# 14chanwa/remotesensingProject

Hardware: AMD Instinct MI355X
Metric: Mpixel*disparity-hypotheses/s (higher is better)
Workload: dtype f32

## Files before the change

### remotesensingproject_amd/csrc/k2_reg.hpp

```cpp
#pragma once

#include "k2_scan.hpp"
#include "k2_taps.hpp"

namespace rslf {

#ifndef RSLF_REG_GB104
#define RSLF_REG_GB104 8
#endif
constexpr int gather_batch(int c) { return c == 1 ? 8 : 4; }
constexpr int kPadSlack = 16;

template <int SPAD, int C, bool PK, bool KONLY>
__device__ __forceinline__ void mean_shift_pass(const float (&R)[PK ? 1 : C][PK ? 1 : SPAD], const f2 (&R2)[PK ? C : 1][PK ? SPAD / 2 : 1],
                                                int S, float kq, const float (&rbar)[C], float (&A)[C], float& B)
{
    static_assert(!KONLY || (C == 1 && !PK), "the K-only pass is written for the scalar one-channel blocks");
    if constexpr (PK) {
        f2 rb2[C];
        const f2 kq2 = {kq, kq};
#pragma unroll
        for (int c = 0; c < C; c++)
            rb2[c] = f2{rbar[c], rbar[c]};
        constexpr int kBlk = (C == 1) ? 8 : 4;
#pragma unroll
        for (int s0 = 0; s0 < SPAD; s0 += kBlk) {
            if (!(s0 < SPAD - kPadSlack || s0 < S))
                continue;
            if constexpr (C == 1) {
                f2 P[4], K[4];
                const f2 r4[4] = {R2[0][s0 / 2], R2[0][s0 / 2 + 1], R2[0][s0 / 2 + 2], R2[0][s0 / 2 + 3]};
                mean_shift_pk_octet(r4, rb2[0], kq2, P, K);
#pragma unroll
                for (int j = 0; j < 4; j++) {
                    A[0] = A[0] + P[j].x;
                    B = B + K[j].x;
                    A[0] = A[0] + P[j].y;
                    B = B + K[j].y;
                }
            } else {
                f2 Pa[3], Pb[3], Ka, Kb;
                const f2 ra[3] = {R2[0][s0 / 2], R2[1][s0 / 2], R2[C - 1][s0 / 2]};
                const f2 rb[3] = {R2[0][s0 / 2 + 1], R2[1][s0 / 2 + 1], R2[C - 1][s0 / 2 + 1]};
                const f2 m[3] = {rb2[0], rb2[C > 1 ? 1 : 0], rb2[C - 1]};
                mean_shift_pk_rgb_quad(ra, rb, m, kq2, Pa, Pb, Ka, Kb);
#pragma unroll
                for (int c = 0; c < C; c++)
                    A[c] = A[c] + Pa[c].x;
                B = B + Ka.x;
#pragma unroll
                for (int c = 0; c < C; c++)
                    A[c] = A[c] + Pa[c].y;
                B = B + Ka.y;
#pragma unroll
                for (int c = 0; c < C; c++)
                    A[c] = A[c] + Pb[c].x;
                B = B + Kb.x;
#pragma unroll
                for (int c = 0; c < C; c++)
                    A[c] = A[c] + Pb[c].y;
                B = B + Kb.y;
            }
        }
    } else if (C == 1) {
#pragma unroll
        for (int s0 = 0; s0 < SPAD; s0 += 4) {
            if (s0 + 4 <= SPAD - kPadSlack || s0 + 4 <= S) {
                if constexpr (KONLY)
                    mean_shift_group4_k(R[0][s0], R[0][s0 + 1], R[0][s0 + 2], R[0][s0 + 3], rbar[0], kq, B);
                else
                    mean_shift_group4(R[0][s0], R[0][s0 + 1], R[0][s0 + 2], R[0][s0 + 3], rbar[0], kq, A[0], B);
            } else {
#pragma unroll
                for (int j = 0; j < 3; j++)
                    if (s0 + j < S) {
                        if constexpr (KONLY)
                            mean_shift_group1_k(R[0][s0 + j], rbar[0], kq, B);
                        else
                            mean_shift_group1(R[0][s0 + j], rbar[0], kq, A[0], B);
                    }
            }
        }
    } else {
#pragma unroll
        for (int s = 0; s < SPAD; s++) {
            if (!(s < SPAD - kPadSlack || s < S))
                continue;
            float q[C];
#pragma unroll
            for (int c = 0; c < C; c++) {
                const float delta = R[c][s] - rbar[c];
                const float tq = kq * delta;
                q[c] = tq * delta;
            }
            float qs = q[0];
            if (C == 3) {
                qs = q[0] + q[C - 1];
                qs = qs + q[C > 1 ? 1 : 0];
            }
            const float K = kernel_weight(qs);
#pragma unroll
            for (int c = 0; c < C; c++) {
                const float pr = R[c][s] * K;
                A[c] = A[c] + pr;
            }
            B = B + K;
        }
    }
}

template <int SPAD, int C, int BATCH>
__device__ __forceinline__ void tap_table_batch(const float* epi, const float* otab, const int* tboff, const f2* tw, unsigned du_bytes,
                                                float uf, int S, int stride_s, bool from_table, int g, int& rowoff, float (&R)[C][SPAD])
{
    float tt[BATCH], om[BATCH], e0[C][BATCH], e1[C][BATCH];
    unsigned bo[BATCH];
    if (from_table) {
#pragma unroll
        for (int j = 0; j < BATCH; j++) {
            const int s = g * BATCH + j;
            bo[j] = (unsigned)tboff[s] + du_bytes;
            const f2 w = tw[s];
            tt[j] = w.x;
            om[j] = w.y;
        }
    } else {
        int ro = rowoff;
#pragma unroll
        for (int j = 0; j < BATCH; j++) {
            const int s = g * BATCH + j;
            tt[j] = 0.0f;
            bo[j] = 0;
            if (s < SPAD - kPadSlack || s < S) {
                const float x = otab[s] + uf;
                tt[j] = lerp_weight(x);
                const int i0 = floor_to_int(x);
                bo[j] = (unsigned)(i0 * C + ro) << 2;
            }
            om[j] = 1.0f - tt[j];
            ro += stride_s;
        }
    }
    rowoff += BATCH * stride_s;
#pragma unroll
    for (int j = 0; j < BATCH; j++) {
        const int s = g * BATCH + j;
#pragma unroll
        for (int c = 0; c < C; c++) {
            e0[c][j] = kSentinel;
            e1[c][j] = 0.0f;
        }
        if (s < SPAD - kPadSlack || s < S) {
            const float* p = (const float*)((const char*)epi + bo[j]);
#pragma unroll
            for (int c = 0; c < C; c++) {
                e0[c][j] = p[c];
                e1[c][j] = p[C + c];
            }
        }
    }
#pragma unroll
    for (int j = 0; j < BATCH; j++) {
        const int s = g * BATCH + j;
#pragma unroll
        for (int c = 0; c < C; c++) {
            const float m0 = om[j] * e0[c][j];
            const float m1 = tt[j] * e1[c][j];
            const float r = m0 + m1;
            R[c][s] = (s < SPAD - kPadSlack || s < S) ? r : kSentinel;
        }
    }
}

template <int SPAD, int C, bool BORDER, bool UNIFORM_D, bool PK, int GB = 0, class BestT = Best<C>, bool LANE_D = false,
          bool TRIM = false, bool TAPS = false>
__device__ __forceinline__ void scan_reg_body(const ScanArgs& a, int v, int u, int d0, int d1, BestT& best,
                                              float* __restrict__ otab, int dlane = 0, int dstep = 1)
{
    static_assert(!LANE_D || !UNIFORM_D, "hypotheses in the lanes: every lane has its own view offsets");
    constexpr int kGatherBatch = GB > 0 ? GB : (C == 1 && !PK && SPAD == 104 && RSLF_REG_GB104 == 13) ? 13 : gather_batch(C);
    static_assert(SPAD % kGatherBatch == 0 && (!PK || kGatherBatch % 2 == 0), "whole batches, whole pairs");
    static_assert(SPAD % 8 == 0, "slot counts are multiples of 8");
    static_assert(!TAPS || (UNIFORM_D && !BORDER && !PK), "the tap table belongs to the interior scalar uniform-D row form");
    const VolView& vol = a.vol;
    const float* epi = vol.row(v, 0);
    const float uf = (float)u;
    const int Um1 = vol.U - 1;
    const unsigned Um1_bits = __float_as_uint((float)Um1);
    const int S = vol.S;
    const int lane = threadIdx.x & 63;
    const long long o = (long long)v * vol.U + u;
    const float dmin = a.dmin_vu ? a.dmin_vu[o] : a.dmin;
    const float dmax = a.dmax_vu ? a.dmax_vu[o] : a.dmax;
    const float range = dmax - dmin;
    const float denom = (float)(a.dim_d - 1);
    const float kq = (C == 1) ? a.k.k1 : a.k.inv_h2;
    const float slope = a.k.slope;
    const int stride_s = (int)vol.stride_s;
    float centre[C];
#pragma unroll
    for (int c = 0; c < C; c++)
        centre[c] = epi[(long long)a.s_hat * vol.stride_s + u * C + c];
    int* const tboff = TAPS ? reinterpret_cast<int*>(otab + SPAD) : nullptr;
    f2* const tw = TAPS ? reinterpret_cast<f2*>(otab + 2 * SPAD) : nullptr;
    int u_first = 0, u_last = 0;
    unsigned du_bytes = 0;
    bool taps_on = false;
    if constexpr (TAPS) {
        u_first = __builtin_amdgcn_readfirstlane(u);
        u_last = __builtin_amdgcn_readlane(u, 63);
        const int du = u - u_first;
        du_bytes = (unsigned)(du * C) << 2;
        taps_on = a.tap_table != 0 && __all(du == min(lane, u_last - u_first));
    }

#pragma unroll 1
    for (int dk = d0; dk < d1; dk += (LANE_D ? dstep : 1)) {
        const int d = LANE_D ? min(dk + dlane, d1 - 1) : dk;
        const float Dd = hypothesis(dmin, range, denom, d);
        float R[PK ? 1 : C][PK ? 1 : SPAD];
        f2 R2[PK ? C : 1][PK ? SPAD / 2 : 1];
        int card = BORDER ? 0 : S;
        float Ss0 = (float)a.s_hat;
        asm volatile("" : "+v"(Ss0));
        int rowoff = 0;
        asm volatile("" : "+s"(rowoff));
        unsigned fastb = 0;
        if (UNIFORM_D) {
            int lane_s = lane, tile_first = u_first, tile_last = u_last;
            if constexpr (TAPS)
                asm volatile("" : "+v"(lane_s), "+s"(tile_first), "+s"(tile_last));
#pragma unroll
            for (int s0 = 0; s0 < SPAD; s0 += 64) {
                const int s = s0 + lane_s;
                float off = (float)(a.s_hat - s) * Dd;
                off = off * slope;
                if (SPAD % 64 == 0 || s < SPAD)
                    otab[s] = off;
                if constexpr (TAPS) {
                    if (taps_on) {
                        const TapEntry e = tap_entry(off, tile_first, tile_last, vol.U, C, __mul24(s, stride_s));
                        if (SPAD % 64 == 0 || s < SPAD) {
                            tboff[s] = e.byteoff;
                            tw[s] = f2{e.t, e.omt};
                        }
                        unsigned long long m = __ballot(e.fast);
                        m &= m >> 1;
                        m &= m >> 2;
                        m &= m >> 4;
                        static_assert(!TAPS || kGatherBatch == 8, "the batch bits are gathered for batches of eight samples");
#pragma unroll
                        for (int k = 0; k < 8; k++)
                            if (s0 + 8 * k < SPAD)
                                fastb |= ((unsigned)(m >> (8 * k)) & 1u) << (s0 / 8 + k);
                    }
                }
            }
            __builtin_amdgcn_wave_barrier();
            if constexpr (TAPS)
                fastb = __builtin_amdgcn_readfirstlane(fastb & (S >= SPAD ? ~0u : (1u << (S / kGatherBatch)) - 1u));
        }
#pragma unroll
        for (int g = 0; g < SPAD / kGatherBatch; g++) {
            if constexpr (TAPS) {
                tap_table_batch<SPAD, C, kGatherBatch>(epi, otab, tboff, tw, du_bytes, uf, S, stride_s, (fastb >> g) & 1u, g, rowoff, R);
            } else {
                float tt[kGatherBatch], e0[C][kGatherBatch], e1[C][kGatherBatch];
                bool ok[kGatherBatch];
#pragma unroll
                for (int j = 0; j < kGatherBatch; j++) {
                    const int s = g * kGatherBatch + j;
                    tt[j] = 0.0f;
                    ok[j] = false;
#pragma unroll
                    for (int c = 0; c < C; c++) {
                        e0[c][j] = kSentinel;
                        e1[c][j] = 0.0f;
                    }
                    if (s < SPAD - kPadSlack || s < S) {
                        float x;
                        if (UNIFORM_D) {
                            x = otab[s];
                        } else {
                            x = (Ss0 - (float)s) * Dd;
                            x = x * slope;
                        }
                        x = x + uf;
                        tt[j] = lerp_weight(x);
                        int i0 = floor_to_int(x);
                        ok[j] = true;
                        if (BORDER) {
                            ok[j] = __float_as_uint(x) <= Um1_bits;
                            i0 = ok[j] ? i0 : 0;
                        }
                        const unsigned byteoff = (unsigned)(i0 * C + rowoff) << 2;
                        const float* p = (const float*)((const char*)epi + byteoff);
#pragma unroll
                        for (int c = 0; c < C; c++) {
                            e0[c][j] = p[c];
                            e1[c][j] = p[C + c];
                        }
                    }
                    rowoff += stride_s;
                }
#pragma unroll
                for (int j = 0; j < kGatherBatch; j++) {
                    const int s = g * kGatherBatch + j;
                    const float omt = 1.0f - tt[j];
#pragma unroll
                    for (int c = 0; c < C; c++) {
                        const float m0 = omt * e0[c][j];
                        const float m1 = tt[j] * e1[c][j];
                        const float r = m0 + m1;
                        float val;
                        if (BORDER)
                            val = ok[j] ? r : kSentinel;
                        else
                            val = (s < SPAD - kPadSlack || s < S) ? r : kSentinel;
                        if constexpr (PK) {
                            if (s & 1)
                                R2[c][s >> 1].y = val;
                            else
                                R2[c][s >> 1].x = val;
                        } else {
                            R[c][s] = val;
                        }
                    }
                    if (BORDER)
                        card += ok[j] ? 1 : 0;
                }
            }
            {
                const int b = g * kGatherBatch;
#pragma unroll
                for (int c = 0; c < C; c++) {
                    if constexpr (PK) {
                        asm volatile("" : "+v"(R2[c][b / 2]), "+v"(R2[c][b / 2 + 1]));
                        if (kGatherBatch == 8)
                            asm volatile("" : "+v"(R2[c][b / 2 + 2]), "+v"(R2[c][b / 2 + 3]));
                        static_assert(!PK || kGatherBatch == 4 || kGatherBatch == 8, "pair pinning is written for 4 and 8");
                    } else if (kGatherBatch != 4 && kGatherBatch != 8) {
#pragma unroll
                        for (int j = 0; j < kGatherBatch; j++)
                            asm volatile("" : "+v"(R[c][b + j]));
                    } else {
                        asm volatile("" : "+v"(R[c][b + 0]), "+v"(R[c][b + 1]), "+v"(R[c][b + 2]), "+v"(R[c][b + 3]));
                        if (kGatherBatch == 8)
                            asm volatile("" : "+v"(R[c][b + kGatherBatch - 4]), "+v"(R[c][b + kGatherBatch - 3]),
                                              "+v"(R[c][b + kGatherBatch - 2]), "+v"(R[c][b + kGatherBatch - 1]));
                    }
                }
                if (BORDER)
                    asm volatile("" : "+s"(rowoff), "+v"(Ss0), "+v"(card));
                else
                    asm volatile("" : "+s"(rowoff), "+v"(Ss0));
            }
        }

        float rbar[C];
#pragma unroll
        for (int c = 0; c < C; c++)
            rbar[c] = centre[c];
        float B = 0.0f;
#pragma unroll 1
        for (int it = 0; it < a.k.n_iter; it++) {
            float A[C];
#pragma unroll
            for (int c = 0; c < C; c++)
                A[c] = 0.0f;
            B = 0.0f;
            if constexpr (TRIM) {
                if (it == a.k.n_iter - 1) {
                    mean_shift_pass<SPAD, C, PK, true>(R, R2, S, kq, rbar, A, B);
                    break;
                }
            }
            mean_shift_pass<SPAD, C, PK, false>(R, R2, S, kq, rbar, A, B);
#pragma unroll
            for (int c = 0; c < C; c++) {
                const float qd = (B != 0.0f) ? (A[c] / B) : 0.0f;
                rbar[c] = (qd > 0.0f) ? qd : 0.0f;
            }
        }
        const float cardf = (float)card;
        float sc = (card != 0) ? (B / cardf) : 0.0f;
        sc = (sc > 0.0f) ? sc : 0.0f;
        if (!LANE_D || dk + dlane < d1)
            best.offer(sc, d, Dd, rbar);
    }
}

template <int C>
struct LastPassRbar {
    __device__ __forceinline__ void operator()(const ScanArgs& a, long long o, float Dd, float (&rbar)[C]) const
    {
        if (a.k.n_iter == 0)
            return;
        const VolView& vol = a.vol;
        const int v = (int)(o / vol.U);
        const int u = (int)(o - (long long)v * vol.U);
        const float* epi = vol.row(v, 0);
        const float uf = (float)u;
        const unsigned Um1_bits = __float_as_uint((float)(vol.U - 1));
        const float kq = (C == 1) ? a.k.k1 : a.k.inv_h2;
        const float Ss0 = (float)a.s_hat;
        const int S = vol.S;
        float A[C];
#pragma unroll
        for (int c = 0; c < C; c++)
            A[c] = 0.0f;
// ... 88 lines not shown
#ifndef RSLF_TAP_TABLE
#define RSLF_TAP_TABLE 1
#endif
constexpr bool scan_reg_tap_table(int spad, int c) { return RSLF_TAP_TABLE && c == 1 && spad == 104 && scan_reg_trim(spad, c); }

template <int SPAD, int C>
using ScanRegRbarFix = std::conditional_t<scan_reg_trim(SPAD, C), LastPassRbar<C>, NoRbarFix>;

template <int SPAD, int C, class BestT>
__device__ __forceinline__ void scan_reg_rows(const ScanArgs& a, int v, int u, int d0, int d1, BestT& best, float* otab)
{
    constexpr bool PK = scan_reg_packed_math(SPAD, C);
    constexpr bool kTaps = scan_reg_tap_table(SPAD, C);
    if (a.dmin_vu) {
        scan_reg_body<SPAD, C, true, false, PK, 0, BestT, false, scan_reg_trim(SPAD, C)>(a, v, u, d0, d1, best, otab);
        return;
    }
    const float max_ds = (float)max(a.s_hat, a.vol.S - 1 - a.s_hat);
    const float range = a.dmax - a.dmin, denom = (float)(a.dim_d - 1);
    const float uf = (float)u, Um1 = (float)(a.vol.U - 1);
    auto interior = [&](int d) -> bool {
        const float reach = max_ds * fabsf(hypothesis(a.dmin, range, denom, d)) * fabsf(a.k.slope) + 2.0f;
        return __all((uf - reach >= 0.0f) && (uf + reach <= Um1));
    };
    int d = d0;
    while (d < d1) {
        const bool in = interior(d);
        int e = d + 1;
        while (e < d1 && interior(e) == in)
            e++;
        if (in)
            scan_reg_body<SPAD, C, false, true, PK, 0, BestT, false, scan_reg_trim(SPAD, C), kTaps>(a, v, u, d, e, best, otab);
        else
            scan_reg_body<SPAD, C, true, true, PK, 0, BestT, false, scan_reg_trim(SPAD, C)>(a, v, u, d, e, best, otab);
        d = e;
    }
}

template <int SPAD, int C>
__global__ __launch_bounds__(64 * kScanWaves) __attribute__((amdgpu_waves_per_eu(scan_reg_waves(SPAD, C), scan_reg_waves(SPAD, C))))
void k2_scan_reg(ScanArgs a)
{
    __shared__ __attribute__((aligned(16))) float s_otab[kScanWaves][SPAD * (scan_reg_tap_table(SPAD, C) ? 4 : 1)];
    float* otab = s_otab[__builtin_amdgcn_readfirstlane(threadIdx.x >> 6)];
    constexpr bool kEpiDyn = false;
    float* const epi_lds = nullptr;
    const int epi_stride = 0;
    using Fix = ScanRegRbarFix<SPAD, C>;
    if constexpr (scan_reg_best_in_lds(SPAD, C)) {
        __shared__ float s_best[kScanWaves][BestLds<C>::kFloats];
        BestLds<C> running(s_best[__builtin_amdgcn_readfirstlane(threadIdx.x >> 6)]);
        RSLF_SCAN_ROW_TILE_FIX((running.init(), scan_reg_rows<SPAD, C>(a, v, u, d0, d1, running, otab), running.load(best)), Fix{})
    } else {
        RSLF_SCAN_ROW_TILE_FIX((scan_reg_rows<SPAD, C>(a, v, u, d0, d1, best, otab)), Fix{})
    }
}

#ifndef RSLF_PACKED_LONG_GB
#define RSLF_PACKED_LONG_GB 4
#endif
constexpr bool packed_long_unit(int spad, int c) { return c == 1 && spad >= 80 && spad <= 128 && spad % RSLF_PACKED_LONG_GB == 0; }
constexpr int packed_waves(int spad, int c) { return packed_long_unit(spad, c) ? 2 : scan_reg_waves(spad + 24, c); }
constexpr int packed_gather_batch(int spad, int c) { return packed_long_unit(spad, c) ? spad / RSLF_PACKED_LONG_GB : 0; }

template <int SPAD, int C>
__global__ __launch_bounds__(64 * kScanWaves) __attribute__((amdgpu_waves_per_eu(packed_waves(SPAD, C), packed_waves(SPAD, C))))
void k2_scan_reg_packed(ScanArgs a)
// ... 48 lines not shown
```

### remotesensingproject_amd/csrc/k2_taps.hpp

```cpp
#pragma once

#include <math.h>
#include <stdint.h>
#include <string.h>

#if defined(__HIPCC__)
#define RSLF_TAPS_FN __host__ __device__ __forceinline__
#else
#define RSLF_TAPS_FN inline
#endif

namespace rslf {

struct TapEntry {
    int byteoff;
    float t, omt;
    bool fast;
};

RSLF_TAPS_FN uint32_t tap_float_bits(float x)
{
#if defined(__HIP_DEVICE_COMPILE__)
    return __float_as_uint(x);
#else
    uint32_t b;
    memcpy(&b, &x, sizeof(b));
    return b;
#endif
}

RSLF_TAPS_FN float tap_fract(float x)
{
#if defined(__HIP_DEVICE_COMPILE__)
    return __builtin_amdgcn_fractf(x);
#else
    return x - floorf(x);
#endif
}
RSLF_TAPS_FN int tap_floor(float x)
{
#if defined(__HIP_DEVICE_COMPILE__)
    int i;
    asm("v_cvt_flr_i32_f32_e32 %0, %1" : "=v"(i) : "v"(x));
    return i;
#else
    return (int)floorf(x);
#endif
}

RSLF_TAPS_FN TapEntry tap_entry(float off, int u_first, int u_last, int U, int C, int row_floats)
{
    const float uf = (float)u_first, ul = (float)u_last;
    const float x_first = off + uf;
    const float x_last = off + ul;
    TapEntry e;
    e.t = tap_fract(x_first);
    const int i0 = tap_floor(x_first);
    e.omt = 1.0f - e.t;
    e.byteoff = (int)((unsigned)(i0 * C + row_floats) << 2);
    const bool inside = x_first > 0.0f && x_last <= (float)(U - 1);
    const bool binade = ((tap_float_bits(x_first) ^ tap_float_bits(x_last)) >> 23) == 0;
    const float back = x_last - ul;
    const bool exact = back == off;
    e.fast = inside && (binade || exact);
    return e;
}

}
```

### remotesensingproject_amd/csrc/rslf_core.hip

```cpp
#include "rslf_internal.hpp"

#include <algorithm>
#include <cmath>

#include "k0_pack.hpp"

using namespace rslf;


namespace rslf {

char* last_error_buffer()
{
    static thread_local char g_err[512] = "";
    return g_err;
}

static std::atomic<int> g_inject[kInjectSites];

bool inject_hit(InjectSite site)
{
    std::atomic<int>& c = g_inject[site];
    int v = c.load(std::memory_order_relaxed);
    while (v > 0)
// ... 184 lines not shown
        (void)hipEventDestroy(ctx->ev1);
    delete ctx;
    return RSLF_OK;
}
RSLF_API_CATCH

extern "C" int rslf_ctx_set_stream(rslf_ctx* ctx, void* hip_stream) RSLF_API_TRY
{
    if (!ctx)
        return fail(RSLF_ERR_INVALID_ARG, "ctx is NULL");
    ctx->stream = (hipStream_t)hip_stream;
    return RSLF_OK;
}
RSLF_API_CATCH

extern "C" int rslf_ctx_set_debug(rslf_ctx* ctx, const char* key, int value) RSLF_API_TRY
{
    if (!ctx || !key)
        return fail(RSLF_ERR_INVALID_ARG, "ctx/key is NULL");
    if (strcmp(key, "force_scan") == 0 && value >= 0 && value <= 2)
        ctx->force_scan = value;
    else if (strcmp(key, "force_groups") == 0 && value >= 0 && value <= 64)
        ctx->force_groups = value;
    else if (strcmp(key, "force_packed") == 0 && value >= -1 && value <= 1)
        ctx->force_packed = value;
    else if (strcmp(key, "px") == 0 && value >= -1 && value <= 1)
        ctx->px_mode = value;
    else if (strcmp(key, "stream_share") == 0 && value >= 0 && value <= 2)
        ctx->stream_share = value;
    else if (strcmp(key, "row_split") == 0 && value >= 0 && value <= 65536)
        ctx->row_split = value;
    else if (strcmp(key, "tap_table") == 0 && (value == 0 || value == 1))
        ctx->tap_table = value;
    else if (strcmp(key, "claim_skip") == 0 && (value == 0 || value == 1))
        ctx->claim_skip = value;
    else if (strcmp(key, "time_all") == 0 && (value == 0 || value == 1)) {
        ctx->time_all = value;
        ctx->ev_used = 0;
    } else if (strcmp(key, "stream_groups") == 0 && value >= 0 && value <= 64)
        ctx->stream_groups = value;
    else if (strcmp(key, "stream_lds_kib") == 0 && value >= 16 && value <= 152) {
        ctx->stream_lds_bytes = (size_t)value << 10;
    } else if (strcmp(key, "staging_kib") == 0 && value >= 0 && value <= 262144)
        ctx->staging_kib = value;
    else
        return fail(RSLF_ERR_INVALID_ARG, "rslf_ctx_set_debug: unknown key or value out of range: %s = %d", key, value);
    return RSLF_OK;
}
RSLF_API_CATCH

extern "C" int rslf_ctx_synchronize(rslf_ctx* ctx) RSLF_API_TRY
{
    if (!ctx)
        return fail(RSLF_ERR_INVALID_ARG, "ctx is NULL");
    HIP_TRY(hipSetDevice(ctx->device));
    HIP_TRY(hipStreamSynchronize(ctx->stream));
    return RSLF_OK;
}
RSLF_API_CATCH


extern "C" int rslf_volume_create(rslf_ctx* ctx, int V, int S, int U, int C, rslf_volume** out) RSLF_API_TRY
{
    if (!ctx || !out)
        return fail(RSLF_ERR_INVALID_ARG, "ctx/out is NULL");
    *out = nullptr;
// ... 474 lines not shown
```

### remotesensingproject_amd/csrc/rslf_internal.hpp

```cpp
#pragma once

#include "../../include/rslf_hip.h"

#include <hip/hip_runtime.h>

#include <atomic>
#include <cstdarg>
#include <cstdio>
#include <cstring>
#include <exception>
#include <functional>
#include <memory>
#include <new>
#include <string>
#include <thread>
#include <vector>

#include "rslf_device.hpp"
#include "rslf_plan.hpp"
#include "rslf_scratch.hpp"


namespace rslf {

// ... 161 lines not shown
    int32_t* lc_idx_vu = nullptr;
    const float* lc_Ce_svu = nullptr;
    const float* lc_dmin_vu = nullptr;
    const float* lc_dmax_vu = nullptr;
    float lc_dmin = 0.0f, lc_dmax = 0.0f;
    int lc_dim_d = 0;
    ScanConsts lc_consts = {};
};

}

struct rslf_ctx {
    int device = 0;
    hipStream_t stream = nullptr;
    rslf::Scratch scratch;
    rslf::SweepState sweep;
    hipEvent_t ev0 = nullptr, ev1 = nullptr;
    bool ev_valid = false;
    int time_all = 0;
    std::vector<hipEvent_t> ev_pool;
    size_t ev_used = 0;
    int last_spad = 0;
    int last_kernel = 0;
    int num_cus = 0;
    int force_scan = 0;
    int force_groups = 0;
    int force_packed = -1;
    int px_mode = -1;
    int stream_groups = 0;
    int stream_share = 1;
    size_t stream_lds_bytes = rslf::plan::kStreamLdsBytes;
    int row_split = 1;
    int tap_table = 1;
    int claim_skip = 1;
    int staging_kib = 0;
};

struct rslf_volume {
    rslf_ctx* ctx = nullptr;
    int device = 0;
    int V = 0, S = 0, U = 0, C = 0, pitch = 0;
    float* base = nullptr;
    size_t bytes = 0;
    float min_value = 0.0f, max_value = 0.0f;
    bool filled = false;
};

struct rslf_multi {
    struct Dev {
        rslf_ctx* ctx = nullptr;
        hipStream_t s_up = nullptr, s_comp = nullptr, s_down = nullptr;
        hipEvent_t done[2] = {nullptr, nullptr};
        rslf_volume* vol[2] = {nullptr, nullptr};
        rslf::DeviceBuf planes[2];
        rslf::PinnedBuf pin[2];
        rslf::DeviceBuf arena;
    };
    std::vector<Dev> devs;
    int chunk_rows = 0;
    std::vector<unsigned char> peer;
};

namespace rslf {

struct StreamScope {
    StreamScope(rslf_ctx* ctx_, hipStream_t stream) : ctx(ctx_), saved(ctx_->stream) { ctx->stream = stream; }
// ... 133 lines not shown
```

### remotesensingproject_amd/csrc/rslf_pile.hip

```cpp
#include "rslf_internal.hpp"

#include <algorithm>
#include <cmath>

#include "k1_edge.hpp"
#include "k2_scan.hpp"
#include "k2_reg.hpp"
#include "k2_stream.hpp"
#include "k3_median.hpp"

using namespace rslf;

static_assert(sizeof(Partial) == plan::kPartialRecordBytes, "rslf_plan.hpp sizes the record scratch");
static_assert(kScanWaves == plan::kScanWavesPerTile, "rslf_plan.hpp shares the hypotheses out over this many waves");


extern "C" int rslf_edge_confidence_pile(rslf_ctx* ctx, const rslf_volume* vol, int s, const rslf_params* p,
                                         float* d_Ce_vu, uint8_t* d_Ce_mask_vu) RSLF_API_TRY
{
    if (!ctx || !vol || !d_Ce_vu || !d_Ce_mask_vu)
        return fail(RSLF_ERR_INVALID_ARG, "NULL argument");
    int rc = check_params(p);
    if (rc)
        return rc;
// ... 122 lines not shown
#define RSLF_C 3
            RSLF_SPAD_LIST_3CH(RSLF_CASE)
#undef RSLF_C
        default:
            break;
        }
    }
#undef RSLF_CASE
    return fail(RSLF_ERR_UNSUPPORTED, "no register scan kernel with %d slots x %d channels", spad, C);
}

static plan::ScanKernelFacts kernel_facts(int S, int C)
{
    const int spad = plan::pick_spad(S, C);
    return plan::ScanKernelFacts{spad ? scan_reg_waves(spad, C) : 0, stream_resident_for(S, C), stream_px_resident_for(S, C)};
}

static plan::ScanRequest scan_request(const rslf_ctx* ctx, int V, int U, int S, int C, int dim_d, bool in_range, bool linear,
                                      bool pixel_ranges, const ScanInputs& in)
{
    plan::ScanRequest rq = {};
    rq.V = V, rq.U = U, rq.S = S, rq.C = C, rq.dim_d = dim_d;
    rq.num_cus = ctx->num_cus;
    rq.ctx_groups = in.groups;
    rq.ctx_packed = in.packed;
    rq.precompacted = in.lists;
    rq.force_groups = ctx->force_groups;
    rq.force_packed = ctx->force_packed;
    rq.px_mode = ctx->px_mode;
    rq.stream_groups = ctx->stream_groups;
    rq.stream_share = ctx->stream_share;
    rq.stream_lds_bytes = ctx->stream_lds_bytes;
    rq.tap_table = ctx->tap_table;
    const bool dense_uniform = !pixel_ranges && !in.packed && ctx->force_packed != 1 && in.lists != ScanInputs::kPackedList;
    plan::choose_scan_kernel(&rq, in_range, linear, ctx->force_scan, dense_uniform, kernel_facts(S, C));
    return rq;
}

int rslf::scan_presize(rslf_ctx* ctx, int S, int U, int C, int dim_d, const rslf_params* p, const int* rows, int n_rows)
{
    const plan::ScanKernelFacts f = kernel_facts(S, C);
    int max_rows = 0;
    size_t recs = 0, tickets = 0;
    for (int i = 0; i < n_rows; i++) {
        max_rows = std::max(max_rows, rows[i]);
        ScanInputs in;
        if (p && plan::fuse_k1_compaction(p->edge_confidence_opening_size, ctx->force_packed, (size_t)rows[i] * U))
            in.lists = ScanInputs::kRowLists;
        const plan::ScanRequest rq = scan_request(ctx, rows[i], U, S, C, dim_d, true, !p || p->interpolation == RSLF_INTERP_LINEAR, false, in);
        const plan::ScanPlan sp = plan::plan_scan(rq, f.nres, f.nres_px);
        recs = std::max(recs, sp.records);
        tickets = std::max(tickets, sp.tickets);
    }
    if (max_rows < 1)
        return RSLF_OK;
    HIP_TRY(hipSetDevice(ctx->device));
    bool tickets_fresh = false;
    int rc = ensure_plane_scratch(ctx, max_rows, U);
    if (rc == RSLF_OK && recs)
        rc = ensure_group_scratch(ctx, recs, tickets, &tickets_fresh);
    if (rc == RSLF_OK && tickets_fresh)
        HIP_TRY(hipStreamSynchronize(ctx->stream));
    return rc;
}

int rslf::sweep_scan_presize(rslf_ctx* ctx, const rslf_volume* vol, int dim_d, const ScanInputs& sparse)
// ... 462 lines not shown
```

### remotesensingproject_amd/csrc/rslf_plan.hpp

```cpp
#pragma once

#include <stddef.h>
#include <stdint.h>

#include <string.h>

#include <algorithm>
#include <cmath>
#include <vector>

#include "../../include/rslf_hip.h"

namespace rslf {

struct MorphElement {
    int k;
    unsigned rows[31];
};

namespace plan {


constexpr int kScanWavesPerTile = 4;
constexpr size_t kPartialRecordBytes = 32;
// ... 547 lines not shown
inline int px_waves(int dim_d)
{
    int best = 0;
    double best_use = 0.0;
    for (int w = 1; w <= kScanWavesPerTile; w *= 2) {
        const int lanes = 64 * w, iters = (dim_d + lanes - 1) / lanes;
        const double use = (double)dim_d / ((double)iters * lanes);
        if (use >= best_use - 1e-12) {
            best_use = use;
            best = w;
        }
    }
    return best_use >= 0.6 ? best : 0;
}

struct ScanRequest {
    int V, U, S, C, dim_d;
    int spad;
    bool use_stream;
    bool use_chip;
    int chip_wave_floats;
    int reg_waves;
    int num_cus;
    int ctx_groups;
    bool ctx_packed;
    int precompacted;
    int force_groups;
    int force_packed;
    int px_mode;
    int stream_groups;
    int stream_share;
    size_t stream_lds_bytes;
    int tap_table;
};

struct ScanPlan {
    int kind;
    int spad;
    int groups;
    bool packed;
    bool packed_adapt;
    int px_waves;
    int tap_table;
    int tile_w;
    int tiles_per_row;
    int rows_per_launch;
    size_t records;
    size_t tickets;
    int stream_nres;
    int stream_park;
    int stream_wave_floats;
    size_t lds_bytes;
};

inline int stream_resident_hi(int C, int nres_1ch, int nres_rgb) { return C == 1 ? nres_1ch : nres_rgb; }

struct ScanKernelFacts {
    int reg_waves;
    int nres;
    int nres_px;
};

inline bool scan_range_ok(float min_value, float max_value) { return min_value >= 0.0f && max_value <= 1.0e6f; }

inline void choose_scan_kernel(ScanRequest* r, bool in_range, bool linear, int force_scan, bool dense_uniform, const ScanKernelFacts& f)
{
// ... 51 lines not shown
    if (r.force_packed >= 0)
        packed = r.force_packed != 0;
    if (n > (size_t)INT32_MAX || r.precompacted == 1)
        packed = false;
    if (r.precompacted == 2)
        packed = true;
    while (groups > 1 && r.dim_d < 2 * kScanWavesPerTile * groups)
        groups /= 2;

    int px_w = 0;
    if (packed && (r.spad || r.use_stream) && !r.use_chip && r.px_mode != 0) {
        px_w = px_waves(r.dim_d);
        if (px_w == 0 && r.px_mode == 1)
            px_w = 1;
    }
    if (px_w && r.use_stream && nres_px >= 0)
        nres = nres_px;
    p.stream_nres = r.use_stream ? nres : 0;
    const int park_early = r.use_stream ? stream_park_for(r.S, r.C, nres, r.stream_lds_bytes) : 0;
    const bool share = r.use_chip ? r.stream_share != 0
                                  : r.use_stream && (r.stream_share == 2 || (r.stream_share == 1 && stream_shares_taps(r.S, nres, park_early)));
    p.tile_w = (share && !packed) ? 63 : 64;
    p.tiles_per_row = p.tile_w == 63 ? std::max(1, (r.U + 61) / 63) : (r.U + p.tile_w - 1) / p.tile_w;
    p.packed_adapt = packed && !r.use_stream && !r.use_chip;
    p.rows_per_launch = r.V;
    if (groups > 1 && !packed) {
        const size_t per_row = (size_t)p.tiles_per_row * groups * 64 * kPartialRecordBytes;
        p.rows_per_launch = (int)std::min<size_t>((size_t)r.V, std::max<size_t>(1, kPartialBudget / per_row));
    }
    if (packed && (r.use_stream || r.use_chip))
        while (groups > 1 && ((n + 63) / 64) * groups * 64 * kPartialRecordBytes > kPartialBudget)
            groups /= 2;
    p.px_waves = px_w;
    p.tap_table = (r.spad && !packed && r.tap_table) ? 1 : 0;
    p.spad = r.spad;
    p.kind = r.spad ? (px_w ? RSLF_SCAN_REG_PX : RSLF_SCAN_REG)
             : r.use_chip ? RSLF_SCAN_CHIP
             : r.use_stream ? (px_w ? RSLF_SCAN_STREAM_PX : RSLF_SCAN_STREAM) : RSLF_SCAN_GENERIC;
    if (px_w) {
        groups = 1;
        p.packed_adapt = false;
    }
    p.groups = groups;
    p.packed = packed;
    p.records = 0;
    p.tickets = 0;
    if (groups > 1) {
        const size_t tiles_all = (n + 63) / 64;
        const size_t tiles_max = !packed ? (size_t)p.rows_per_launch * p.tiles_per_row
                                         : p.packed_adapt ? std::min<size_t>(tiles_all, kPackedItemTarget / 2) : tiles_all;
        p.records = (packed && p.packed_adapt) ? std::min<size_t>(tiles_all * groups, kPackedItemTarget) * 64 : tiles_max * groups * 64;
        p.tickets = tiles_max;
    }
    p.stream_park = 0;
    p.stream_wave_floats = 0;
    p.lds_bytes = 0;
    if (r.use_stream) {
        const size_t s4 = ((size_t)r.S + 3) & ~(size_t)3;
        const int park = park_early;
        p.stream_park = park;
        p.stream_wave_floats = (int)(s4 + (size_t)park * r.C * 64);
        p.stream_wave_floats = std::max(p.stream_wave_floats, 2 * (64 + (3 + r.C) * 32));
        p.lds_bytes = (size_t)kScanWavesPerTile * p.stream_wave_floats * sizeof(float);
    }
    if (r.use_chip) {
        p.stream_wave_floats = r.chip_wave_floats;
        p.lds_bytes = (size_t)kScanWavesPerTile * r.chip_wave_floats * sizeof(float);
// ... 209 lines not shown
```

### remotesensingproject_amd/depth.py

```python
from __future__ import annotations

import atexit
import copy
import ctypes as C
import sys
from dataclasses import dataclass
from typing import Optional, Sequence

import numpy as np
import torch

from . import _lib
from ._lib import RslfParams, RslfStats, RslfVolumeDesc, check


class Interpolation1DLinear:
    mode = 0


class Interpolation1DNearestNeighbour:

    def __init__(self, as_built: bool = False):
        self.mode = 2 if as_built else 1

# ... 33 lines not shown
            v = getattr(self, "par_" + f)
            setattr(p, f, int(v) if isinstance(getattr(p, f), int) else float(v))
        return p


LINE_CONF_OFF, LINE_CONF_AS_BUILT, LINE_CONF_GATE = 0, 1, 2


def require_no_line_confidence(parameters, who: str) -> None:
    if parameters is not None and int(parameters.par_line_confidence_mode) != LINE_CONF_OFF:
        raise ValueError("%s: par_line_confidence_mode=%d is not built here (one-device Depth2DComputer only)"
                         % (who, int(parameters.par_line_confidence_mode)))


class Context:

    def __init__(self, device: int | torch.device | None = None):
        if device is None:
            device = torch.cuda.current_device()
        self.device = torch.device("cuda", device) if isinstance(device, int) else torch.device(device)
        h = C.c_void_p()
        check(_lib.lib().rslf_ctx_create(self.device.index or 0, C.byref(h)), "rslf_ctx_create")
        self._h = h
        self.use_current_stream()

    def use_current_stream(self) -> None:
        s = torch.cuda.current_stream(self.device).cuda_stream
        check(_lib.lib().rslf_ctx_set_stream(self._h, C.c_void_p(s)), "rslf_ctx_set_stream")

    def synchronize(self) -> None:
        check(_lib.lib().rslf_ctx_synchronize(self._h), "rslf_ctx_synchronize")

    _DEBUG_DEFAULTS = dict(force_scan=0, force_groups=0, force_packed=-1, px=-1, stream_share=1, stream_groups=0, stream_lds_kib=80,
                           claim_skip=1, time_all=0, row_split=1, staging_kib=0, tap_table=1)
    _FORCE_SCAN = {None: 0, "auto": 0, "generic": 1, "stream": 2}

    def set_debug(self, **hooks) -> None:
        for k, v in hooks.items():
            if k == "force_scan" and not isinstance(v, int):
                v = self._FORCE_SCAN[v or None]
            check(_lib.lib().rslf_ctx_set_debug(self._h, k.encode(), int(v)), "rslf_ctx_set_debug(%s)" % k)

    def reset_debug(self) -> None:
        self.set_debug(**self._DEBUG_DEFAULTS)

    def last_scan_kernel_ms(self) -> float:
        ms = C.c_float()
        check(_lib.lib().rslf_last_scan_kernel_ms(self._h, C.byref(ms)), "rslf_last_scan_kernel_ms")
        return float(ms.value)

    def scan_time_total_ms(self) -> tuple[float, int]:
        ms, n = C.c_float(), C.c_int()
        check(_lib.lib().rslf_scan_time_total_ms(self._h, C.byref(ms), C.byref(n)), "rslf_scan_time_total_ms")
        return float(ms.value), int(n.value)

    def close(self) -> None:
        if getattr(self, "_h", None) and not sys.is_finalizing():
            _lib.lib().rslf_ctx_destroy(self._h)
        self._h = None

    def __del__(self):
        try:
            self.close()
        except Exception:
            pass


# ... 1071 lines not shown
```

Before: 8132.

## Taper gather batch rounds to issue more loads early in tap-table path

Introduces a compile-time gather schedule that groups several 8-sample batches into one round for the SPAD=104 single-channel tap-table path (3,3,2,2,1,1,1). Early rounds issue more loads before any use, which gives more memory-level parallelism, and later rounds shrink. It also marks padded slots past S as fast so their batches take the table path. The risks are higher register pressure from the larger rounds and possible spills in the early portion.

Result: no change. 8183 (median of 6 runs) (+0.6%).

```diff
diff --git a/remotesensingproject_amd/csrc/k2_reg.hpp b/remotesensingproject_amd/csrc/k2_reg.hpp
--- a/remotesensingproject_amd/csrc/k2_reg.hpp
+++ b/remotesensingproject_amd/csrc/k2_reg.hpp
@@ -1,15 +1,59 @@
 #pragma once
+
+#include <utility>
 
 #include "k2_scan.hpp"
 #include "k2_taps.hpp"
 
 namespace rslf {
 
-#ifndef RSLF_REG_GB104
-#define RSLF_REG_GB104 8
-#endif
 constexpr int gather_batch(int c) { return c == 1 ? 8 : 4; }
 constexpr int kPadSlack = 16;
+
+#ifndef RSLF_GATHER_TAPER
+#define RSLF_GATHER_TAPER 1
+#endif
+constexpr int kMaxGatherBatches = 64;
+struct GatherSchedule {
+    int batches;
+    int round_first[kMaxGatherBatches];
+    int round_count[kMaxGatherBatches];
+    int max_count;
+    bool uniform;
+};
+constexpr GatherSchedule gather_rounds(int batches, const int* rounds)
+{
+    GatherSchedule g{};
+    g.batches = batches;
+    g.max_count = 1;
+    g.uniform = true;
+    int b = 0;
+    for (int r = 0; b < batches; r++) {
+        const int n = rounds ? rounds[r] : 1;
+        for (int i = 0; i < n; i++) {
+            g.round_first[b + i] = b;
+            g.round_count[b + i] = n;
+        }
+        g.max_count = n > g.max_count ? n : g.max_count;
+        g.uniform = g.uniform && n == 1;
+        b += n;
+    }
+    return g;
+}
+enum GatherForm { kGatherOther, kGatherTaps, kGatherBorder, kGatherRange };
+constexpr GatherSchedule gather_schedule(int spad, int c, int batch, GatherForm form)
+{
+    constexpr int k104[] = {3, 3, 2, 2, 1, 1, 1, 0};
+    const bool tapered = ((RSLF_GATHER_TAPER & 1) && form == kGatherTaps) || ((RSLF_GATHER_TAPER & 2) && form == kGatherBorder) ||
+                         ((RSLF_GATHER_TAPER & 4) && form == kGatherRange);
+    if (tapered && c == 1 && spad == 104 && batch == 8)
+        return gather_rounds(spad / batch, k104);
+    return gather_rounds(spad / batch, nullptr);
+}
+template <int SPAD, int C, int BATCH, GatherForm FORM>
+struct GatherRounds {
+    static constexpr GatherSchedule v = gather_schedule(SPAD, C, BATCH, FORM);
+};
 
 template <int SPAD, int C, bool PK, bool KONLY>
 __device__ __forceinline__ void mean_shift_pass(const float (&R)[PK ? 1 : C][PK ? 1 : SPAD], const f2 (&R2)[PK ? C : 1][PK ? SPAD / 2 : 1],
@@ -109,41 +153,60 @@
     }
 }
 
-template <int SPAD, int C, int BATCH>
-__device__ __forceinline__ void tap_table_batch(const float* epi, const float* otab, const int* tboff, const f2* tw, unsigned du_bytes,
-                                                float uf, int S, int stride_s, bool from_table, int g, int& rowoff, float (&R)[C][SPAD])
-{
-    float tt[BATCH], om[BATCH], e0[C][BATCH], e1[C][BATCH];
-    unsigned bo[BATCH];
-    if (from_table) {
-#pragma unroll
-        for (int j = 0; j < BATCH; j++) {
-            const int s = g * BATCH + j;
-            bo[j] = (unsigned)tboff[s] + du_bytes;
-            const f2 w = tw[s];
-            tt[j] = w.x;
-            om[j] = w.y;
-        }
-    } else {
-        int ro = rowoff;
-#pragma unroll
-        for (int j = 0; j < BATCH; j++) {
-            const int s = g * BATCH + j;
-            tt[j] = 0.0f;
-            bo[j] = 0;
-            if (s < SPAD - kPadSlack || s < S) {
-                const float x = otab[s] + uf;
-                tt[j] = lerp_weight(x);
-                const int i0 = floor_to_int(x);
-                bo[j] = (unsigned)(i0 * C + ro) << 2;
-            }
-            om[j] = 1.0f - tt[j];
-            ro += stride_s;
-        }
-    }
-    rowoff += BATCH * stride_s;
-#pragma unroll
-    for (int j = 0; j < BATCH; j++) {
+#ifndef RSLF_TAP_PAD_SLOTS
+#define RSLF_TAP_PAD_SLOTS 1
+#endif
+template <int SPAD, bool ONE_BATCH_ROUNDS>
+__device__ __forceinline__ int round_slot(int s) { return ONE_BATCH_ROUNDS ? s : (s < SPAD ? s : SPAD - 1); }
+
+template <int SPAD, int C, int BATCH, int KMAX, int K>
+__device__ __forceinline__ void tap_table_entries(const float* otab, const int* tboff, const f2* tw, unsigned du_bytes, float uf, int S,
+                                                  int stride_s, unsigned fastb, int g, int gn, int& rowoff, float (&tt)[KMAX * BATCH],
+                                                  float (&om)[KMAX * BATCH], unsigned (&bo)[KMAX * BATCH])
+{
+    if (KMAX == 1 || K < gn) {
+        if ((fastb >> (g + K)) & 1u) {
+#pragma unroll
+            for (int j = K * BATCH; j < (K + 1) * BATCH; j++) {
+                const int s = g * BATCH + j;
+                bo[j] = (unsigned)tboff[s] + du_bytes;
+                const f2 w = tw[s];
+                tt[j] = w.x;
+                om[j] = w.y;
+            }
+        } else {
+            int ro = rowoff;
+#pragma unroll
+            for (int j = K * BATCH; j < (K + 1) * BATCH; j++) {
+                const int s = g * BATCH + j;
+                tt[j] = 0.0f;
+                bo[j] = 0;
+                if (s < SPAD - kPadSlack || s < S) {
+                    const float x = otab[s] + uf;
+                    tt[j] = lerp_weight(x);
+                    const int i0 = floor_to_int(x);
+                    bo[j] = (unsigned)(i0 * C + ro) << 2;
+                }
+                om[j] = 1.0f - tt[j];
+                ro += stride_s;
+            }
+        }
+        rowoff += BATCH * stride_s;
+    }
+}
+template <int SPAD, int C, int BATCH, int KMAX, int... K>
+__device__ __forceinline__ void tap_table_round(const float* epi, const float* otab, const int* tboff, const f2* tw, unsigned du_bytes,
+                                                float uf, int S, int stride_s, unsigned fastb, int g, int gn, int& rowoff,
+                                                float (&R)[C][SPAD], std::integer_sequence<int, K...>)
+{
+    constexpr int N = KMAX * BATCH;
+    float tt[N], om[N], e0[C][N], e1[C][N];
+    unsigned bo[N];
+    (tap_table_entries<SPAD, C, BATCH, KMAX, K>(otab, tboff, tw, du_bytes, uf, S, stride_s, fastb, g, gn, rowoff, tt, om, bo), ...);
+#pragma unroll
+    for (int j = 0; j < N; j++) {
+        if (KMAX > 1 && j >= gn * BATCH)
+            continue;
         const int s = g * BATCH + j;
 #pragma unroll
         for (int c = 0; c < C; c++) {
@@ -160,14 +223,16 @@
         }
     }
 #pragma unroll
-    for (int j = 0; j < BATCH; j++) {
+    for (int j = 0; j < N; j++) {
+        if (KMAX > 1 && j >= gn * BATCH)
+            continue;
         const int s = g * BATCH + j;
 #pragma unroll
         for (int c = 0; c < C; c++) {
             const float m0 = om[j] * e0[c][j];
             const float m1 = tt[j] * e1[c][j];
             const float r = m0 + m1;
-            R[c][s] = (s < SPAD - kPadSlack || s < S) ? r : kSentinel;
+            R[c][round_slot<SPAD, KMAX == 1>(s)] = (s < SPAD - kPadSlack || s < S) ? r : kSentinel;
         }
     }
 }
@@ -178,8 +243,14 @@
                                               float* __restrict__ otab, int dlane = 0, int dstep = 1)
 {
     static_assert(!LANE_D || !UNIFORM_D, "hypotheses in the lanes: every lane has its own view offsets");
-    constexpr int kGatherBatch = GB > 0 ? GB : (C == 1 && !PK && SPAD == 104 && RSLF_REG_GB104 == 13) ? 13 : gather_batch(C);
+    constexpr int kGatherBatch = GB > 0 ? GB : gather_batch(C);
     static_assert(SPAD % kGatherBatch == 0 && (!PK || kGatherBatch % 2 == 0), "whole batches, whole pairs");
+    static_assert(SPAD / kGatherBatch <= kMaxGatherBatches, "the schedule has a place for every batch");
+    constexpr GatherForm kForm = (PK || LANE_D || GB > 0) ? kGatherOther : TAPS ? kGatherTaps : !BORDER ? kGatherOther
+                                 : UNIFORM_D ? kGatherBorder : kGatherRange;
+    using Rounds = GatherRounds<SPAD, C, kGatherBatch, kForm>;
+    constexpr bool kOneBatchRounds = Rounds::v.uniform;
+    constexpr int kRoundMax = Rounds::v.max_count * kGatherBatch;
     static_assert(SPAD % 8 == 0, "slot counts are multiples of 8");
     static_assert(!TAPS || (UNIFORM_D && !BORDER && !PK), "the tap table belongs to the interior scalar uniform-D row form");
     const VolView& vol = a.vol;
@@ -244,7 +315,7 @@
                             tboff[s] = e.byteoff;
                             tw[s] = f2{e.t, e.omt};
                         }
-                        unsigned long long m = __ballot(e.fast);
+                        unsigned long long m = __ballot(e.fast || (RSLF_TAP_PAD_SLOTS && s >= S));
                         m &= m >> 1;
                         m &= m >> 2;
                         m &= m >> 4;
@@ -258,17 +329,25 @@
             }
             __builtin_amdgcn_wave_barrier();
             if constexpr (TAPS)
-                fastb = __builtin_amdgcn_readfirstlane(fastb & (S >= SPAD ? ~0u : (1u << (S / kGatherBatch)) - 1u));
+                fastb = __builtin_amdgcn_readfirstlane(
+                    fastb & (S >= SPAD ? ~0u : (1u << ((S + (RSLF_TAP_PAD_SLOTS ? kGatherBatch - 1 : 0)) / kGatherBatch)) - 1u));
         }
 #pragma unroll
         for (int g = 0; g < SPAD / kGatherBatch; g++) {
+            if (!kOneBatchRounds && Rounds::v.round_first[g] != g)
+                continue;
+            const int gn = kOneBatchRounds ? 1 : Rounds::v.round_count[g];
             if constexpr (TAPS) {
-                tap_table_batch<SPAD, C, kGatherBatch>(epi, otab, tboff, tw, du_bytes, uf, S, stride_s, (fastb >> g) & 1u, g, rowoff, R);
+                tap_table_round<SPAD, C, kGatherBatch, Rounds::v.max_count>(epi, otab, tboff, tw, du_bytes, uf, S, stride_s, fastb, g, gn,
+                                                                            rowoff, R,
+                                                                            std::make_integer_sequence<int, Rounds::v.max_count>{});
             } else {
-                float tt[kGatherBatch], e0[C][kGatherBatch], e1[C][kGatherBatch];
-                bool ok[kGatherBatch];
-#pragma unroll
-                for (int j = 0; j < kGatherBatch; j++) {
+                float tt[kRoundMax], e0[C][kRoundMax], e1[C][kRoundMax];
+                bool ok[kRoundMax];
+#pragma unroll
+                for (int j = 0; j < kRoundMax; j++) {
+                    if (!kOneBatchRounds && j >= gn * kGatherBatch)
+                        continue;
                     const int s = g * kGatherBatch + j;
                     tt[j] = 0.0f;
                     ok[j] = false;
@@ -304,7 +383,9 @@
                     rowoff += stride_s;
                 }
 #pragma unroll
-                for (int j = 0; j < kGatherBatch; j++) {
+                for (int j = 0; j < kRoundMax; j++) {
+                    if (!kOneBatchRounds && j >= gn * kGatherBatch)
+                        continue;
                     const int s = g * kGatherBatch + j;
                     const float omt = 1.0f - tt[j];
 #pragma unroll
@@ -319,19 +400,22 @@
                             val = (s < SPAD - kPadSlack || s < S) ? r : kSentinel;
                         if constexpr (PK) {
                             if (s & 1)
-                                R2[c][s >> 1].y = val;
+                                R2[c][round_slot<SPAD, kOneBatchRounds>(s) >> 1].y = val;
                             else
-                                R2[c][s >> 1].x = val;
+                                R2[c][round_slot<SPAD, kOneBatchRounds>(s) >> 1].x = val;
                         } else {
-                            R[c][s] = val;
+                            R[c][round_slot<SPAD, kOneBatchRounds>(s)] = val;
                         }
                     }
                     if (BORDER)
                         card += ok[j] ? 1 : 0;
                 }
             }
-            {
-                const int b = g * kGatherBatch;
+#pragma unroll
+            for (int k = 0; k < Rounds::v.max_count; k++) {
+                if (!kOneBatchRounds && k >= gn)
+                    continue;
+                const int b = round_slot<SPAD, kOneBatchRounds>((g + k) * kGatherBatch);
 #pragma unroll
                 for (int c = 0; c < C; c++) {
                     if constexpr (PK) {
@@ -350,11 +434,11 @@
                                               "+v"(R[c][b + kGatherBatch - 2]), "+v"(R[c][b + kGatherBatch - 1]));
                     }
                 }
-                if (BORDER)
-                    asm volatile("" : "+s"(rowoff), "+v"(Ss0), "+v"(card));
-                else
-                    asm volatile("" : "+s"(rowoff), "+v"(Ss0));
-            }
+            }
+            if (BORDER)
+                asm volatile("" : "+s"(rowoff), "+v"(Ss0), "+v"(card));
+            else
+                asm volatile("" : "+s"(rowoff), "+v"(Ss0));
         }
 
         float rbar[C];
```

## Skip fully out-of-bounds sample batches in border tiles using a live mask

Applied to the files above, without the earlier changes.

Extends the tap-table path to border tiles. A per-hypothesis live bitmask marks samples whose shifted view falls entirely outside the image for the whole 64-pixel tile. Batches of eight dead samples skip the gather and are filled with the sentinel, and the mean-shift passes skip dead groups of four. The aim is to cut wasted gathers and kernel arithmetic at image borders, at the cost of extra ballots, scalar mask registers and larger border code.

Measured after the change: 8237 before, 8287 after (median of 6 runs). No clear change (+0.6%).

```diff
diff --git a/remotesensingproject_amd/csrc/k2_reg.hpp b/remotesensingproject_amd/csrc/k2_reg.hpp
--- a/remotesensingproject_amd/csrc/k2_reg.hpp
+++ b/remotesensingproject_amd/csrc/k2_reg.hpp
@@ -11,11 +11,14 @@
 constexpr int gather_batch(int c) { return c == 1 ? 8 : 4; }
 constexpr int kPadSlack = 16;
 
-template <int SPAD, int C, bool PK, bool KONLY>
+constexpr int live_words(int spad) { return (spad + 31) / 32; }
+template <int SPAD, int C, bool PK, bool KONLY, bool MASKED = false>
 __device__ __forceinline__ void mean_shift_pass(const float (&R)[PK ? 1 : C][PK ? 1 : SPAD], const f2 (&R2)[PK ? C : 1][PK ? SPAD / 2 : 1],
-                                                int S, float kq, const float (&rbar)[C], float (&A)[C], float& B)
+                                                int S, float kq, const float (&rbar)[C], float (&A)[C], float& B,
+                                                const unsigned* live = nullptr)
 {
     static_assert(!KONLY || (C == 1 && !PK), "the K-only pass is written for the scalar one-channel blocks");
+    static_assert(!MASKED || (C == 1 && !PK), "the masked pass is written for the scalar one-channel blocks");
     if constexpr (PK) {
         f2 rb2[C];
         const f2 kq2 = {kq, kq};
@@ -63,9 +66,21 @@
             }
         }
     } else if (C == 1) {
+        unsigned lw[live_words(SPAD)];
+        if constexpr (MASKED) {
+#pragma unroll
+            for (int w = 0; w < live_words(SPAD); w++) {
+                lw[w] = live[w];
+                asm volatile("" : "+s"(lw[w]));
+            }
+        }
 #pragma unroll
         for (int s0 = 0; s0 < SPAD; s0 += 4) {
-            if (s0 + 4 <= SPAD - kPadSlack || s0 + 4 <= S) {
+            if constexpr (MASKED) {
+                if ((lw[s0 >> 5] & (0xfu << (s0 & 31))) == 0)
+                    continue;
+            }
+            if (MASKED || s0 + 4 <= SPAD - kPadSlack || s0 + 4 <= S) {
                 if constexpr (KONLY)
                     mean_shift_group4_k(R[0][s0], R[0][s0 + 1], R[0][s0 + 2], R[0][s0 + 3], rbar[0], kq, B);
                 else
@@ -181,7 +196,7 @@
     constexpr int kGatherBatch = GB > 0 ? GB : (C == 1 && !PK && SPAD == 104 && RSLF_REG_GB104 == 13) ? 13 : gather_batch(C);
     static_assert(SPAD % kGatherBatch == 0 && (!PK || kGatherBatch % 2 == 0), "whole batches, whole pairs");
     static_assert(SPAD % 8 == 0, "slot counts are multiples of 8");
-    static_assert(!TAPS || (UNIFORM_D && !BORDER && !PK), "the tap table belongs to the interior scalar uniform-D row form");
+    static_assert(!TAPS || (UNIFORM_D && !PK && C == 1), "the tap table belongs to the scalar uniform-D row form");
     const VolView& vol = a.vol;
     const float* epi = vol.row(v, 0);
     const float uf = (float)u;
@@ -212,7 +227,10 @@
         const int du = u - u_first;
         du_bytes = (unsigned)(du * C) << 2;
         taps_on = a.tap_table != 0 && __all(du == min(lane, u_last - u_first));
-    }
+        if constexpr (BORDER)
+            taps_on = taps_on && (a.tap_table & 2) != 0;
+    }
+    constexpr bool kMasked = BORDER && TAPS;
 
 #pragma unroll 1
     for (int dk = d0; dk < d1; dk += (LANE_D ? dstep : 1)) {
@@ -226,6 +244,7 @@
         int rowoff = 0;
         asm volatile("" : "+s"(rowoff));
         unsigned fastb = 0;
+        unsigned live[kMasked ? live_words(SPAD) : 1];
         if (UNIFORM_D) {
             int lane_s = lane, tile_first = u_first, tile_last = u_last;
             if constexpr (TAPS)
@@ -237,14 +256,20 @@
                 off = off * slope;
                 if (SPAD % 64 == 0 || s < SPAD)
                     otab[s] = off;
-                if constexpr (TAPS) {
+                if constexpr (kMasked) {
+                    const bool out = (taps_on && tap_outside(off, tile_first, tile_last, vol.U)) || s >= S;
+                    const unsigned long long m = ~__ballot(out);
+                    live[s0 / 32] = (unsigned)m;
+                    if (s0 + 32 < SPAD)
+                        live[s0 / 32 + 1] = (unsigned)(m >> 32);
+                } else if constexpr (TAPS) {
                     if (taps_on) {
                         const TapEntry e = tap_entry(off, tile_first, tile_last, vol.U, C, __mul24(s, stride_s));
                         if (SPAD % 64 == 0 || s < SPAD) {
                             tboff[s] = e.byteoff;
                             tw[s] = f2{e.t, e.omt};
                         }
-                        unsigned long long m = __ballot(e.fast);
+                        unsigned long long m = __ballot(e.fast || s >= S);
                         m &= m >> 1;
                         m &= m >> 2;
                         m &= m >> 4;
@@ -257,12 +282,23 @@
                 }
             }
             __builtin_amdgcn_wave_barrier();
-            if constexpr (TAPS)
-                fastb = __builtin_amdgcn_readfirstlane(fastb & (S >= SPAD ? ~0u : (1u << (S / kGatherBatch)) - 1u));
+            if constexpr (TAPS && !BORDER)
+                fastb = __builtin_amdgcn_readfirstlane(fastb);
         }
 #pragma unroll
         for (int g = 0; g < SPAD / kGatherBatch; g++) {
-            if constexpr (TAPS) {
+            static_assert(!kMasked || kGatherBatch == 8, "the out test is written for batches of eight samples");
+            bool out_batch = false;
+            if constexpr (kMasked) {
+                out_batch = (live[(g * 8) >> 5] & (0xffu << ((g * 8) & 31))) == 0;
+                if (out_batch) {
+#pragma unroll
+                    for (int j = 0; j < kGatherBatch; j++)
+                        R[0][g * kGatherBatch + j] = kSentinel;
+                }
+            }
+            if (kMasked && out_batch) {
+            } else if constexpr (TAPS && !BORDER) {
                 tap_table_batch<SPAD, C, kGatherBatch>(epi, otab, tboff, tw, du_bytes, uf, S, stride_s, (fastb >> g) & 1u, g, rowoff, R);
             } else {
                 float tt[kGatherBatch], e0[C][kGatherBatch], e1[C][kGatherBatch];
@@ -350,6 +386,8 @@
                                               "+v"(R[c][b + kGatherBatch - 2]), "+v"(R[c][b + kGatherBatch - 1]));
                     }
                 }
+                if constexpr (kMasked)
+                    rowoff = (g + 1) * kGatherBatch * stride_s;
                 if (BORDER)
                     asm volatile("" : "+s"(rowoff), "+v"(Ss0), "+v"(card));
                 else
@@ -371,11 +409,17 @@
             B = 0.0f;
             if constexpr (TRIM) {
                 if (it == a.k.n_iter - 1) {
-                    mean_shift_pass<SPAD, C, PK, true>(R, R2, S, kq, rbar, A, B);
+                    if constexpr (kMasked)
+                        mean_shift_pass<SPAD, C, PK, true, true>(R, R2, S, kq, rbar, A, B, live);
+                    else
+                        mean_shift_pass<SPAD, C, PK, true>(R, R2, S, kq, rbar, A, B);
                     break;
                 }
             }
-            mean_shift_pass<SPAD, C, PK, false>(R, R2, S, kq, rbar, A, B);
+            if constexpr (kMasked)
+                mean_shift_pass<SPAD, C, PK, false, true>(R, R2, S, kq, rbar, A, B, live);
+            else
+                mean_shift_pass<SPAD, C, PK, false>(R, R2, S, kq, rbar, A, B);
 #pragma unroll
             for (int c = 0; c < C; c++) {
                 const float qd = (B != 0.0f) ? (A[c] / B) : 0.0f;
@@ -530,7 +574,7 @@
         if (in)
             scan_reg_body<SPAD, C, false, true, PK, 0, BestT, false, scan_reg_trim(SPAD, C), kTaps>(a, v, u, d, e, best, otab);
         else
-            scan_reg_body<SPAD, C, true, true, PK, 0, BestT, false, scan_reg_trim(SPAD, C)>(a, v, u, d, e, best, otab);
+            scan_reg_body<SPAD, C, true, true, PK, 0, BestT, false, scan_reg_trim(SPAD, C), kTaps>(a, v, u, d, e, best, otab);
         d = e;
     }
 }
diff --git a/remotesensingproject_amd/csrc/k2_taps.hpp b/remotesensingproject_amd/csrc/k2_taps.hpp
--- a/remotesensingproject_amd/csrc/k2_taps.hpp
+++ b/remotesensingproject_amd/csrc/k2_taps.hpp
@@ -16,6 +16,8 @@
     int byteoff;
     float t, omt;
     bool fast;
+    bool inside;
+    bool outside;
 };
 
 RSLF_TAPS_FN uint32_t tap_float_bits(float x)
@@ -48,6 +50,16 @@
 #endif
 }
 
+RSLF_TAPS_FN bool tap_valid(float x, uint32_t Um1_bits) { return tap_float_bits(x) <= Um1_bits; }
+
+RSLF_TAPS_FN bool tap_all_inside(float x_first, float x_last, int U) { return x_first >= 0.0f && x_last <= (float)(U - 1); }
+RSLF_TAPS_FN bool tap_all_outside(float x_first, float x_last, int U) { return x_last < 0.0f || x_first > (float)(U - 1); }
+
+RSLF_TAPS_FN bool tap_outside(float off, int u_first, int u_last, int U)
+{
+    return tap_all_outside(off + (float)u_first, off + (float)u_last, U);
+}
+
 RSLF_TAPS_FN TapEntry tap_entry(float off, int u_first, int u_last, int U, int C, int row_floats)
 {
     const float uf = (float)u_first, ul = (float)u_last;
@@ -63,6 +75,8 @@
     const float back = x_last - ul;
     const bool exact = back == off;
     e.fast = inside && (binade || exact);
+    e.inside = tap_all_inside(x_first, x_last, U);
+    e.outside = tap_all_outside(x_first, x_last, U);
     return e;
 }
 
diff --git a/remotesensingproject_amd/csrc/rslf_core.hip b/remotesensingproject_amd/csrc/rslf_core.hip
--- a/remotesensingproject_amd/csrc/rslf_core.hip
+++ b/remotesensingproject_amd/csrc/rslf_core.hip
@@ -240,6 +240,8 @@
         ctx->row_split = value;
     else if (strcmp(key, "tap_table") == 0 && (value == 0 || value == 1))
         ctx->tap_table = value;
+    else if (strcmp(key, "tap_border") == 0 && (value == 0 || value == 1))
+        ctx->tap_border = value;
     else if (strcmp(key, "claim_skip") == 0 && (value == 0 || value == 1))
         ctx->claim_skip = value;
     else if (strcmp(key, "time_all") == 0 && (value == 0 || value == 1)) {
diff --git a/remotesensingproject_amd/csrc/rslf_internal.hpp b/remotesensingproject_amd/csrc/rslf_internal.hpp
--- a/remotesensingproject_amd/csrc/rslf_internal.hpp
+++ b/remotesensingproject_amd/csrc/rslf_internal.hpp
@@ -217,6 +217,7 @@
     size_t stream_lds_bytes = rslf::plan::kStreamLdsBytes;
     int row_split = 1;
     int tap_table = 1;
+    int tap_border = 1;
     int claim_skip = 1;
     int staging_kib = 0;
 };
diff --git a/remotesensingproject_amd/csrc/rslf_pile.hip b/remotesensingproject_amd/csrc/rslf_pile.hip
--- a/remotesensingproject_amd/csrc/rslf_pile.hip
+++ b/remotesensingproject_amd/csrc/rslf_pile.hip
@@ -178,6 +178,7 @@
     rq.stream_share = ctx->stream_share;
     rq.stream_lds_bytes = ctx->stream_lds_bytes;
     rq.tap_table = ctx->tap_table;
+    rq.tap_border = ctx->tap_border;
     const bool dense_uniform = !pixel_ranges && !in.packed && ctx->force_packed != 1 && in.lists != ScanInputs::kPackedList;
     plan::choose_scan_kernel(&rq, in_range, linear, ctx->force_scan, dense_uniform, kernel_facts(S, C));
     return rq;
diff --git a/remotesensingproject_amd/csrc/rslf_plan.hpp b/remotesensingproject_amd/csrc/rslf_plan.hpp
--- a/remotesensingproject_amd/csrc/rslf_plan.hpp
+++ b/remotesensingproject_amd/csrc/rslf_plan.hpp
@@ -603,6 +603,7 @@
     int stream_share;
     size_t stream_lds_bytes;
     int tap_table;
+    int tap_border;
 };
 
 struct ScanPlan {
@@ -720,7 +721,7 @@
         while (groups > 1 && ((n + 63) / 64) * groups * 64 * kPartialRecordBytes > kPartialBudget)
             groups /= 2;
     p.px_waves = px_w;
-    p.tap_table = (r.spad && !packed && r.tap_table) ? 1 : 0;
+    p.tap_table = (r.spad && !packed && r.tap_table) ? (r.tap_border ? 3 : 1) : 0;
     p.spad = r.spad;
     p.kind = r.spad ? (px_w ? RSLF_SCAN_REG_PX : RSLF_SCAN_REG)
              : r.use_chip ? RSLF_SCAN_CHIP
diff --git a/remotesensingproject_amd/depth.py b/remotesensingproject_amd/depth.py
--- a/remotesensingproject_amd/depth.py
+++ b/remotesensingproject_amd/depth.py
@@ -89,7 +89,7 @@
         check(_lib.lib().rslf_ctx_synchronize(self._h), "rslf_ctx_synchronize")
 
     _DEBUG_DEFAULTS = dict(force_scan=0, force_groups=0, force_packed=-1, px=-1, stream_share=1, stream_groups=0, stream_lds_kib=80,
-                           claim_skip=1, time_all=0, row_split=1, staging_kib=0, tap_table=1)
+                           claim_skip=1, time_all=0, row_split=1, staging_kib=0, tap_table=1, tap_border=1)
     _FORCE_SCAN = {None: 0, "auto": 0, "generic": 1, "stream": 2}
 
     def set_debug(self, **hooks) -> None:
```
